# williamyang1991/VToonify

Hardware: AMD Instinct MI355X
Metric: frames/sec at 1024x1024 VToonify-D inference (higher is better)
Workload: dtype bf16

## Files before the change

### __graft_entry__.py

```python
from __future__ import annotations

import json
import os
import sys

REPO = os.path.dirname(os.path.abspath(__file__))
if REPO not in sys.path:
    sys.path.insert(0, REPO)


def build() -> None:
    from vtoonify_amd import build as vbuild
    path = vbuild.build(verbose=False)
    assert os.path.exists(path), path
    sys.path.insert(0, os.path.join(REPO, "tests"))
    from emu import build_emu
    build_emu.build()
    import torch
    from vtoonify_amd import _lib
    import ctypes
    lib = ctypes.CDLL(path)
    for sym in _lib.EXPORTED_SYMBOLS:
        getattr(lib, sym)
    import vtoonify_amd.op
    import vtoonify_amd.vtoonify
    print(f"[build] {path} ok ({len(_lib.EXPORTED_SYMBOLS)} symbols)")


def smoke() -> None:
    import numpy as np
    import torch

    from oracle import vtoonify_oracle as O
    from vtoonify_amd import _lib, synth
    from vtoonify_amd.engine import VToonifyEngine

    assert torch.cuda.is_available(), "smoke() needs a GPU"
# ... 27 lines not shown
```

### include/vtoonify_amd.h

```cpp
#ifndef VTOONIFY_AMD_H
#define VTOONIFY_AMD_H

#include <stdint.h>

#ifdef __cplusplus
extern "C" {
#endif

#define VT_ABI_VERSION 5

enum { VT_F32 = 0, VT_BF16 = 1, VT_F16 = 2,
       VT_F32X3 = 3,
       VT_F64 = 4 };
enum { VT_OK = 0, VT_ERR_ARG = 1, VT_ERR_UNSUPPORTED = 2, VT_ERR_LAUNCH = 3 };

enum { VT_ACT_NONE = 0, VT_ACT_LRELU = 1, VT_ACT_RELU_TANH = 2, VT_ACT_SIGMOID = 3, VT_ACT_TANH = 4  };
enum { VT_OUT_NHWC = 0, VT_OUT_NCHW = 1 };

typedef void* vt_stream;

int vt_abi_version(void);
const char* vt_last_error(void);
const char* vt_build_target(void);

// ... 159 lines not shown
int vt_coords_from_flow(float* coords, const float* flow, int n, int h, int w, vt_stream stream);
int vt_convex_upsample(float* out, const float* flow, const float* mask, int n, int h, int w, vt_stream stream);

int vt_nchw_to_nhwc(void* out, int ld_out, const void* in, int n, int c, int hw,
                    int in_dtype, int out_dtype, vt_stream stream);
int vt_nhwc_to_nchw(void* out, const void* in, int ld_in, int n, int c, int hw,
                    int in_dtype, int out_dtype, vt_stream stream);

int vt_mfma_selftest(float* c, const void* a, const void* b, int dtype, vt_stream stream);

#ifdef __cplusplus
}
#endif

#include "vtoonify_amd_prepass.h"
#endif
```

### vtoonify_amd/_lib.py

```python
from __future__ import annotations

import ctypes as C
import os

HERE = os.path.dirname(os.path.abspath(__file__))
DEFAULT_LIB = os.path.join(HERE, "lib", "libvtoonify_amd.so")

ABI_VERSION = 5
VT_F32, VT_BF16, VT_F16 = 0, 1, 2
VT_F64 = 4
VT_F32X3 = 3
ACT_NONE, ACT_LRELU, ACT_RELU_TANH, ACT_SIGMOID, ACT_TANH = 0, 1, 2, 3, 4
OUT_NHWC, OUT_NCHW = 0, 1


class VtError(RuntimeError):
    pass


class ConvDesc(C.Structure):
    _fields_ = [
        ("src0", C.c_void_p), ("src1", C.c_void_p),
        ("c0", C.c_int32), ("c1", C.c_int32), ("ld0", C.c_int32), ("ld1", C.c_int32),
        ("n", C.c_int32), ("h", C.c_int32), ("w", C.c_int32),
# ... 104 lines not shown
                                 C.c_int, C.c_int, C.c_int, C.c_int, C.c_void_p]),
    "vt_nchw_to_nhwc": (C.c_int, [C.c_void_p, C.c_int, C.c_void_p, C.c_int, C.c_int, C.c_int, C.c_int,
                                  C.c_int, C.c_void_p]),
    "vt_nhwc_to_nchw": (C.c_int, [C.c_void_p, C.c_void_p, C.c_int, C.c_int, C.c_int, C.c_int, C.c_int,
                                  C.c_int, C.c_void_p]),
    "vt_mfma_selftest": (C.c_int, [C.c_void_p, C.c_void_p, C.c_void_p, C.c_int, C.c_void_p]),
}

EXPORTED_SYMBOLS = tuple(_SIGS)

_PREPASS_SIGS = {
    "vt_frame_ingest2x": (C.c_int, [C.c_void_p] * 4 + [C.c_int] * 4 + [C.c_void_p]),
}
PREPASS_SYMBOLS = tuple(_PREPASS_SIGS)

_lib = None
_lib_path = None


def _bind(path: str):
    import torch
    lib = C.CDLL(path)
    for name, (res, args) in {**_SIGS, **_PREPASS_SIGS}.items():
        fn = getattr(lib, name)
        fn.restype = res
        fn.argtypes = args
    if lib.vt_abi_version() != ABI_VERSION:
        raise VtError(f"{path}: ABI version {lib.vt_abi_version()} != {ABI_VERSION}")
    return lib


def use_library(path: str):
    global _lib, _lib_path
    _lib = _bind(path)
    _lib_path = path
    return _lib


# ... 35 lines not shown
```

### vtoonify_amd/build.py

```python
from __future__ import annotations

import os
import shutil
import subprocess
import sys
from concurrent.futures import ThreadPoolExecutor

HERE = os.path.dirname(os.path.abspath(__file__))
CSRC = os.path.join(HERE, "csrc")
LIBDIR = os.path.join(HERE, "lib")
LIBNAME = "libvtoonify_amd.so"
SOURCES = ["capi.hip", "fused_bias_act.hip", "upfirdn2d.hip", "style_ops.hip", "conv_igemm.hip",
           "norm_glue.hip", "frame_io.hip", "parsing_glue.hip", "raft_corr.hip", "flow_ops.hip"]
ARCH = "gfx950"
FLAGS = [f"--offload-arch={ARCH}", "-O3", "-std=c++17", "-fPIC", "-fno-gpu-rdc", "-Wno-unused-result", "-ffp-contract=off",
         "-fno-slp-vectorize"]


def hipcc_path() -> str:
    for cand in (os.environ.get("HIPCC"), shutil.which("hipcc"), "/opt/rocm/bin/hipcc"):
        if cand and os.path.exists(cand):
            return cand
    raise RuntimeError("hipcc not found (ROCm toolchain required to build libvtoonify_amd.so)")


def lib_path() -> str:
    return os.path.join(LIBDIR, LIBNAME)


def _deps(src: str):
    hdrs = [os.path.join(CSRC, f) for f in os.listdir(CSRC) if f.endswith(".hpp")]
    hdrs.append(os.path.join(os.path.dirname(HERE), "include", "vtoonify_amd.h"))
    return [src] + hdrs


def _stale(target: str, deps) -> bool:
    if not os.path.exists(target):
        return True
    t = os.path.getmtime(target)
    return any(os.path.getmtime(d) > t for d in deps)


def _stamp(hipcc: str, flags) -> str:
    import hashlib
    try:
        ver = subprocess.run([hipcc, "--version"], capture_output=True, text=True).stdout
    except OSError:
# ... 74 lines not shown
```

### vtoonify_amd/csrc/conv_igemm.hip

```cpp
#include <stdlib.h>
#include <type_traits>
#include <utility>

#include "vt_common.hpp"

namespace {

#ifdef VT_EMU
typedef emu_f32x4 f32x4;
#else
typedef float f32x4 __attribute__((ext_vector_type(4)));
typedef __bf16 bf16x8_t __attribute__((ext_vector_type(8)));
typedef _Float16 f16x8_t __attribute__((ext_vector_type(8)));
#endif

static inline int slab_ld(int cout_total) { return (cout_total + 31) / 32 * 32; }
constexpr int64_t VT_TICKET_BYTES = 16384;

struct ConvArgs {
    const void* src0;
    const void* src1;
    const void* wgt;
    const float* bias;
    const float* slope_vec;
// ... 22 lines not shown
    int force_generic;
    StatRec* stats_part;
    int post_relu;
    const void* wstream;
    float* tile_stats;
    const float* in_tile_stats;
    int in_stats_dil;
    const float* in_gb;
    int in_ld_gb;
    const float* up_fir;
    int rgb_only;
    int in_absdiff;
    int x3;
    int blk_pm, blk_cn;
    int stride_x, dil_x;
};

static inline bool axes_equal(const ConvArgs& a) { return a.stride_x == a.stride && a.dil_x == a.dil && a.pad_x == a.pad; }

template <typename T>
struct Mma;
template <>
struct Mma<bf16_t> {
    static __device__ __forceinline__ void run(f32x4& acc, const u128& a, const u128& b) {
#ifdef VT_EMU
        emu_bf16x8 av, bv;
        memcpy(&av, &a, 16);
        memcpy(&bv, &b, 16);
        acc = emu_mfma_f32_16x16x32_bf16(av, bv, acc);
#else
// ... 2519 lines not shown
extern "C" int vt_conv2d(const vt_conv_desc* d, vt_stream stream) {
    ConvArgs a;
    const int rc = fill_args(d, a);
    if (rc != VT_OK) return rc;
    const int64_t wsf = (d->splitk_ws && d->splitk_ws_bytes > VT_TICKET_BYTES) ? (d->splitk_ws_bytes - VT_TICKET_BYTES) / 4 : 0;
    g_stats_emitted = false;
    a.x3 = d->dtype == VT_F32X3;
    const int rcl = d->dtype == VT_F16    ? dispatch<f16_t>(a, d->tile_hint, wsf, stream)
                    : d->dtype == VT_BF16 ? dispatch<bf16_t>(a, d->tile_hint, wsf, stream)
                                          : dispatch<float>(a, d->tile_hint, wsf, stream);
    if (rcl != VT_OK || !a.stats_part || g_stats_emitted || d->splitk_phase == 1) return rcl;
    return vt_internal_instnorm_partial(a.stats_part, d->out, d->ld_out, d->n, d->out_h * d->out_w, d->cout,
                                        d->dtype == VT_F32X3 ? VT_F32 : d->dtype, stream);
}

extern "C" int vt_conv2d_tile(const vt_conv_desc* d) {
    ConvArgs a;
    if (fill_args(d, a) != VT_OK) return -1;
    a.force_generic = d->tile_hint >= 1000000000 || !axes_equal(a);
    const int64_t wsf = (d->splitk_ws && d->splitk_ws_bytes > VT_TICKET_BYTES) ? (d->splitk_ws_bytes - VT_TICKET_BYTES) / 4 : 0;
    const TilePlan t = plan_of(d, a, wsf);
    int kind = t.kind;
    if (kind == 0) {
        GldsArgs g;
        const bool glds = d->dtype == VT_F16    ? glds_eligible<f16_t>(a, g)
                          : d->dtype == VT_BF16 ? glds_eligible<bf16_t>(a, g)
                                                : glds_eligible<float>(a, g);
        kind = glds ? 2 : 0;
    }
    int bm = t.bm, bn = t.bn;
// ... 95 lines not shown
```

### vtoonify_amd/csrc/conv_thin.hpp

```cpp
#pragma once

constexpr int TH_TW = 8;
constexpr int TH_NW = 4;
constexpr int TH_MAXF = 7;
constexpr int TH_COLS = 32;
constexpr int TH_PADC = 4;

template <typename T>
static bool thin_eligible(const ConvArgs& a) {
    constexpr int KSTEP = 4 * (16 / (int)sizeof(T));
    if (a.force_generic || !axes_equal(a) || a.transposed || a.rgb_w || a.stats_part || a.tile_stats || a.in_tile_stats || a.up_fir || a.slope_vec)
        return false;
    if (a.in_scale && !a.in_shift) return false;
    if ((a.in_scale || a.in_absdiff) && !(a.taps == 9 && a.taps * a.coutT <= 16)) return false;
    if (a.out_layout != VT_OUT_NCHW || a.phases != 1 || a.stride != 1 || a.dil != 1) return false;
    if (!((a.taps == 9 && a.kw == 3 && a.pad == 1) || (a.taps == 1 && a.pad == 0))) return false;
    if (a.coutT < 1 || a.coutT > 3 || a.taps * a.coutT > TH_COLS) return false;
    if (a.in_absdiff ? (a.c1 != a.c0 || !a.src1 || a.ld1 % (16 / (int)sizeof(T)) != 0 || (uintptr_t)a.src1 % 16 != 0) : a.c1 != 0)
        return false;
    if (a.c0 % KSTEP != 0 || a.ld0 % (16 / (int)sizeof(T)) != 0) return false;
    if (a.Ho != a.H || a.Wo != a.W) return false;
    if ((uintptr_t)a.src0 % 16 != 0 || (uintptr_t)a.wgt % 16 != 0) return false;
    return (int64_t)a.N * a.H * a.W * a.ld0 * (int64_t)sizeof(T) < ((int64_t)1 << 40);
}

__device__ __forceinline__ int thin_tile_of_block() {
    const int nb = (int)gridDim.x, b = (int)blockIdx.x;
    const int q = nb >> 3, r = nb & 7;
    const int xcd = b & 7, idx = b >> 3;
    return (xcd < r ? xcd * (q + 1) : r * (q + 1) + (xcd - r) * q) + idx;
}

template <typename T, int KS, int NB, bool PRO = false>
__global__ void __launch_bounds__(TH_NW * 64) conv_thin_kernel(const ConvArgs p) {
    constexpr int VEC = 16 / (int)sizeof(T);
    constexpr int KSTEP = 4 * VEC;
    constexpr int PW = TH_TW + KS - 1;
    constexpr int NPIX = PW * PW;
    constexpr int NF = (NPIX + 15) / 16;
    constexpr int TAPS = KS * KS;
    constexpr int UNR = KS == 3 ? 3 : 4;
    __shared__ __attribute__((aligned(16))) float dpart[TH_NW][NF * 16][16 * NB + TH_PADC];

    const int tid = threadIdx.x;
    const int lane = tid & 63;
    const int wave = vt_uniform(tid >> 6) & (TH_NW - 1);
    const int q = lane >> 4, l15 = lane & 15;
    const int tiles_x = (p.W + TH_TW - 1) / TH_TW, tiles_y = (p.H + TH_TW - 1) / TH_TW;
    const int tile = thin_tile_of_block();
    const int img = tile / (tiles_x * tiles_y);
    const int trem = tile - img * (tiles_x * tiles_y);
    const int y0 = (trem / tiles_x) * TH_TW, x0 = (trem % tiles_x) * TH_TW;
    const int ncols = TAPS * p.coutT;

    const T* src = (const T*)p.src0;
    const T* oth = (const T*)p.src1;
    int64_t poff[NF], qoff[PRO ? NF : 1];
// ... 113 lines not shown
#pragma unroll
            for (int f = 0; f < NF; ++f) affine(fa[f], poff[f] >= 0, scv, shv, &fo[f]);
#pragma unroll
            for (int f = 0; f < NF; ++f)
#pragma unroll
                for (int b = 0; b < NB; ++b) Mma<T>::run(acc[f][b], fw[b], fa[f]);
        }
    }
#pragma unroll
    for (int f = 0; f < NF; ++f)
#pragma unroll
        for (int b = 0; b < NB; ++b) {
            float v4[4] = {acc[f][b][0], acc[f][b][1], acc[f][b][2], acc[f][b][3]};
            st128(&dpart[wave][f * 16 + l15][b * 16 + q * 4], pack16<float>(v4));
        }
    __syncthreads();

    const int opix = tid & 63, co = tid >> 6;
    const int oy = opix / TH_TW, ox = opix - oy * TH_TW;
    const int gy = y0 + oy, gx = x0 + ox;
    if (co >= p.coutT || gy >= p.H || gx >= p.W) return;
    float s = 0.0f;
#pragma unroll
    for (int tap = 0; tap < TAPS; ++tap) {
        const int ky = tap / KS, kx = tap - ky * KS;
        const int pp = (oy + ky) * PW + ox + kx;
        float t = 0.0f;
#pragma unroll
        for (int w = 0; w < TH_NW; ++w) t += dpart[w][pp][tap * p.coutT + co];
        s += t;
    }
    const float ga = p.gain_alpha * (p.alpha_dev ? p.alpha_dev[0] : 1.0f);
    const float v = conv_finish(p, s, p.bias ? p.bias[co] : 0.0f, ga, p.slope);
    const int64_t HoWo = (int64_t)p.H * p.W;
    const int64_t off = ((int64_t)img * p.cout + co) * HoWo + (int64_t)gy * p.W + gx;
    const float* rs = (const float*)p.resid;
    ((float*)p.out)[off] = post_act(p, v + (rs ? p.beta * rs[off] : 0.0f));
}

constexpr int TH16 = 16;
constexpr int TH16_NW = 4;

template <typename T, int KS, int NB, bool PRO = false>
__global__ void __launch_bounds__(TH16_NW * 64) conv_thin16_kernel(const ConvArgs p) {
    constexpr int VEC = 16 / (int)sizeof(T);
    constexpr int KSTEP = 4 * VEC;
    constexpr int PW = TH16 + KS - 1;
    constexpr int NPIX = PW * PW;
    constexpr int NF = (NPIX + 15) / 16;
    constexpr int FPW = (NF + TH16_NW - 1) / TH16_NW;
    constexpr int TAPS = KS * KS;
    constexpr int UNR = 2;
    __shared__ __attribute__((aligned(16))) float dt[NF * 16][16 * NB + TH_PADC];

    const int tid = threadIdx.x;
    const int lane = tid & 63;
    const int wave = vt_uniform(tid >> 6) & (TH16_NW - 1);
    const int q = lane >> 4, l15 = lane & 15;
    const int tiles_x = (p.W + TH16 - 1) / TH16, tiles_y = (p.H + TH16 - 1) / TH16;
    const int tile = thin_tile_of_block();
    const int img = tile / (tiles_x * tiles_y);
    const int trem = tile - img * (tiles_x * tiles_y);
    const int y0 = (trem / tiles_x) * TH16, x0 = (trem % tiles_x) * TH16;
    const int ncols = TAPS * p.coutT;

    const T* src = (const T*)p.src0;
    const T* oth = (const T*)p.src1;
    int64_t poff[FPW], qoff[PRO ? FPW : 1];
// ... 105 lines not shown
                    for (int b = 0; b < NB; ++b) Mma<T>::run(acc[i][b], fw[u][b], fa[u][i]);
            }
        }
    }
#pragma unroll
    for (int i = 0; i < FPW; ++i) {
        const int f = wave + TH16_NW * i;
        if (f < NF) {
#pragma unroll
            for (int b = 0; b < NB; ++b) {
                float v4[4] = {acc[i][b][0], acc[i][b][1], acc[i][b][2], acc[i][b][3]};
                st128(&dt[f * 16 + l15][b * 16 + q * 4], pack16<float>(v4));
            }
        }
    }
    __syncthreads();
    if (tid >= TH16 * TH16) return;
    const int oy = tid / TH16, ox = tid - oy * TH16;
    const int gy = y0 + oy, gx = x0 + ox;
    if (gy >= p.H || gx >= p.W) return;
    const float ga = p.gain_alpha * (p.alpha_dev ? p.alpha_dev[0] : 1.0f);
    const int64_t HoWo = (int64_t)p.H * p.W;
    const float* rs = (const float*)p.resid;
    for (int co = 0; co < p.coutT; ++co) {
        float s = 0.0f;
#pragma unroll
        for (int tap = 0; tap < TAPS; ++tap) {
            const int ky = tap / KS, kx = tap - ky * KS;
            s += dt[(oy + ky) * PW + ox + kx][tap * p.coutT + co];
        }
        const float v = conv_finish(p, s, p.bias ? p.bias[co] : 0.0f, ga, p.slope);
        const int64_t off = ((int64_t)img * p.cout + co) * HoWo + (int64_t)gy * p.W + gx;
        ((float*)p.out)[off] = post_act(p, v + (rs ? p.beta * rs[off] : 0.0f));
    }
}

static bool thin16_wanted(const ConvArgs& a) {
    return a.taps == 9 && (int64_t)vt_cdiv(a.H, TH16) * vt_cdiv(a.W, TH16) >= 256;
}

template <typename T>
int launch_thin(const ConvArgs& a, vt_stream stream) {
    ConvArgs args = a;
    args.splitk = 1;
    args.kps = 0;
    const int64_t blocks = (int64_t)a.N * vt_cdiv(a.H, TH_TW) * vt_cdiv(a.W, TH_TW);
    if (blocks >= ((int64_t)1 << 31)) {
        vt_set_error("vt_conv2d: too many tiles");
        return VT_ERR_ARG;
    }
    const bool two = a.taps * a.coutT > 16;
    if ((a.in_scale || a.in_absdiff) && (a.taps != 9 || two)) {
        vt_set_error("vt_conv2d: in_scale / in_absdiff on a thin conv need a 3x3 kernel with 9 * cout <= 16");
        return VT_ERR_UNSUPPORTED;
    }
    if (thin16_wanted(a)) {
        const unsigned b16 = (unsigned)((int64_t)a.N * vt_cdiv(a.H, TH16) * vt_cdiv(a.W, TH16));
        if (a.in_scale || a.in_absdiff) {
            auto k = conv_thin16_kernel<T, 3, 1, true>;
            VT_LAUNCH(k, dim3(b16), dim3(TH16_NW * 64), stream, args);
        } else if (two) {
            auto k = conv_thin16_kernel<T, 3, 2>;
            VT_LAUNCH(k, dim3(b16), dim3(TH16_NW * 64), stream, args);
        } else {
            auto k = conv_thin16_kernel<T, 3, 1>;
            VT_LAUNCH(k, dim3(b16), dim3(TH16_NW * 64), stream, args);
        }
        return vt_check_launch("vt_conv2d(thin, 16x16)");
    }
    if (a.in_scale || a.in_absdiff) {
        auto k = conv_thin_kernel<T, 3, 1, true>;
        VT_LAUNCH(k, dim3((unsigned)blocks), dim3(TH_NW * 64), stream, args);
    } else if (a.taps == 9 && two) {
        auto k = conv_thin_kernel<T, 3, 2>;
        VT_LAUNCH(k, dim3((unsigned)blocks), dim3(TH_NW * 64), stream, args);
    } else if (a.taps == 9) {
        auto k = conv_thin_kernel<T, 3, 1>;
        VT_LAUNCH(k, dim3((unsigned)blocks), dim3(TH_NW * 64), stream, args);
    } else {
        auto k = conv_thin_kernel<T, 1, 1>;
        VT_LAUNCH(k, dim3((unsigned)blocks), dim3(TH_NW * 64), stream, args);
    }
    return vt_check_launch("vt_conv2d(thin)");
// ... 2 lines not shown
```

### vtoonify_amd/engine.py

```python
from __future__ import annotations

import ctypes as C
import math
import os
from typing import Dict, List, Optional, Tuple

import torch

from . import _lib
from . import kernels as K
from ._lib import ACT_LRELU, ACT_NONE, ACT_RELU_TANH, OUT_NCHW, OUT_NHWC

SQRT2 = math.sqrt(2.0)
N_LATENT = 18
_DIL = {1: 4, 2: 4, 3: 2, 4: 2, 5: 1, 6: 1}
FEM_HDR = 64


def _pad8(c: int) -> int:
    return (c + 7) // 8 * 8


class _Plan:
    def __init__(self):
# ... 2 lines not shown
        self.enc_ops: List[Tuple] = []
        self.gen_ops: List[Tuple] = []
        self.keep: list = []
        self.masks: List[torch.Tensor] = []
        self.graphs: dict = {}
        self.convs: list = []


class VToonifyEngine:
    supports_borrow = True

    def __init__(self, state_dict: Dict[str, torch.Tensor], backbone: str = "dualstylegan",
                 in_size: int = 256, dtype: torch.dtype = torch.bfloat16,
                 device: Optional[torch.device] = None, cache_styles: bool = False,
                 tile_hints: Optional[Dict[str, int]] = None, style_gate: bool = False, x3: bool = False,
                 fuse_rgb128: bool = True):
        assert backbone in ("dualstylegan", "toonify")
        assert dtype in (torch.bfloat16, torch.float16, torch.float32)
        self.backbone = backbone
        self.dual = backbone == "dualstylegan"
        self.in_size = in_size
        self.dtype = dtype
        self.dt = K.dt_code(dtype)
        self.x3 = bool(x3) and dtype == torch.float32
        self.dt_conv = K.VT_F32X3 if self.x3 else self.dt
        self.h16 = dtype in (torch.bfloat16, torch.float16)
        self.precision = ({torch.bfloat16: "bf16", torch.float16: "fp16"}[dtype] if self.h16 else
                          ("fp32x3" if self.x3 else "fp32_exact"))
        self.esz = 2 if self.h16 else 4
        any_t = next(iter(state_dict.values()))
        self.device = torch.device(device) if device is not None else any_t.device
        if self.device.type == "cuda" and self.device.index is None:
            self.device = torch.device("cuda", torch.cuda.current_device())
        self.lib = _lib.lib()
        if self.device.type != "cuda" and not _lib.is_emulation():
            raise _lib.VtError("VToonifyEngine needs a GPU device (no CPU path)")
        self.cache_styles = cache_styles
        self.fuse_rgb128 = bool(fuse_rgb128)
        self.style_gate = bool(style_gate)
        self.graph_first = os.environ.get("VT_GRAPH_FIRST", "1") != "0"
        self.use_upblur = True
        self.tile_hints: Dict[str, int] = dict(tile_hints or {})
        if not self.tile_hints and os.environ.get("VT_TILE_HINTS"):
            import json
            with open(os.environ["VT_TILE_HINTS"]) as f:
                self.tile_hints = {k: int(v) for k, v in json.load(f).items()}
        self.sd = {k: v.detach().to(self.device, torch.float32).contiguous() for k, v in state_dict.items()}
        self.g = "generator.generator." if self.dual else "generator."
        self.n_down = 0
        while f"encoder.{self.n_down}.0.weight" in self.sd:
            self.n_down += 1
        self.n_fuse = sum(1 for lvl in range(5) if 2 ** (5 + lvl) <= in_size)
        import collections
# ... 69 lines not shown
        t = torch.empty(shape, dtype=dtype or self.dtype, device=self.device)
        plan.bufs[name] = t
        return t

    @staticmethod
    def conv_signature(d) -> str:
        return (f"{d.h}x{d.w}:{d.c0 + d.c1}->{d.cout * d.phases}:k{d.kh}s{d.stride}d{d.dil}p{d.phases}"
                + (":nchw" if d.out_layout == OUT_NCHW else "") + (":up" if d.up_fir else ""))

    def _apply_hint(self, d):
        h = self.tile_hints.get(self.conv_signature(d))
        if h:
            d.tile_hint = int(h)
        return d

    def _op_conv(self, ops, plan, ref_macs=None, branch=0, join=False, **kw):
        wt = kw.get("weight")
        if isinstance(wt, torch.Tensor) and wt.data_ptr() in self._wstream:
            kw["weight_stream"] = self._wstream[wt.data_ptr()]
        d = self._apply_hint(K.make_conv_desc(dtype=self.dt_conv, **kw))
        plan.keep.append(d)
        cin = d.c0 + d.c1
        m = d.n * d.out_h * d.out_w
        cout_t = d.cout * d.phases
        macs = m * cout_t * d.kh * d.kw * cin if ref_macs is None else ref_macs
        osz = 4 if d.out_dtype == K.VT_F32 else 2
        nbytes = (d.n * d.h * d.w * cin * self.esz + cout_t * d.kh * d.kw * cin * self.esz +
                  m * cout_t * osz * (2 if d.resid else 1))
        info = {"name": "conv", "kernel": "conv_igemm", "flops": 2 * macs, "bytes": nbytes, "cin": cin,
                "cout": cout_t, "m": m, "k": d.kh * d.kw * cin, "hw": (d.out_h, d.out_w),
                "sig": self.conv_signature(d)}
        if branch:
            info["branch"] = branch
        if join:
            info["join"] = True
        plan.convs.append((d, info, ops, len(ops)))
        ops.append((self.lib.vt_conv2d, (C.byref(d),), info))

    def _conv_kind(self, **kw) -> int:
        wt = kw.get("weight")
        if isinstance(wt, torch.Tensor) and wt.data_ptr() in self._wstream:
            kw["weight_stream"] = self._wstream[wt.data_ptr()]
        d = self._apply_hint(K.make_conv_desc(dtype=self.dt_conv, **kw))
        d.splitk_ws, d.splitk_ws_bytes = 1 << 20, 1 << 40
        tile = self.lib.vt_conv2d_tile(C.byref(d))
        return tile // 100000000 if tile >= 0 else -1

    def _op_linear(self, ops, y, ld_y, x, ld_x, W, b, rows, w_scale=1.0, b_scale=1.0, act=ACT_NONE,
                   slope=0.2, gain=1.0):
        out_dim, in_dim = W.shape
        ops.append((self.lib.vt_linear,
# ... 262 lines not shown
        plan.feat = (feat, cf, h, w)
        skip = self._buf(plan, "skip_enc", (B, 3, h, w), f32)
        self._op_conv(ops, plan, src0=feat, c0=cf, ld0=cf, n=B, h=h, w=w, out_h=h, out_w=w,
                      weight=self.w["enc_rgb"], cout=3, kh=1, kw=1, bias=sd[f"encoder.{self.n_down + 1}.bias"],
                      out=skip, ld_out=0, out_layout=OUT_NCHW, out_dtype=K.VT_F32, branch=1)
        plan.skip_enc = skip

        ops = plan.gen_ops
        out, co = feat, cf
        for lvl in range(5):
            hw = h * w
            if lvl < self.n_fuse:
                f_e, ce, he, we = feats[lvl]
                assert (he, we) == (h, w) and ce == co, "encoder/generator size mismatch (H, W must be multiples of 8)"
                fem = self._buf(plan, f"fem{lvl}", (B, h, w, co + FEM_HDR))
                mask = None
                if self.dual:
                    sc = self._buf(plan, f"fsc{lvl}", (B, 2 * co), f32)
                    sh = self._buf(plan, f"fsh{lvl}", (B, 2 * co), f32)
                    ws = self._buf(plan, f"fws{lvl}", (max(K.instnorm_ws_bytes(B, hw, 2 * co), 16),), torch.uint8)
                    gb = plan.bufs[f"gb.fus.{lvl}"]
                    ops.append((lib.vt_instnorm_stats,
                                (C.c_void_p(sc.data_ptr()), C.c_void_p(sh.data_ptr()), C.c_void_p(out.data_ptr()), co,
                                 C.c_void_p(f_e.data_ptr()), co, B, hw, co, C.c_void_p(gb.data_ptr()),
                                 0 if ns == 1 else gb.shape[1], C.c_void_p(ws.data_ptr()), dt),
                                {"name": "instnorm", "kernel": "instnorm_stats", "flops": 0,
                                 "bytes": 2 * B * hw * co * self.esz}))
                    mask = self._buf(plan, f"mask{lvl}", (B, 1, h, w), f32)
                    mask_kw = dict(n=B, h=h, w=w, out_h=h, out_w=w, weight=self.w[f"fusion_out.{lvl}.conv2"], cout=1,
                                   kh=3, kw=3, pad=1, bias=sd[f"fusion_out.{lvl}.conv2.bias"], act=ACT_RELU_TANH,
                                   out=mask, ld_out=0, out_layout=OUT_NCHW, out_dtype=K.VT_F32)
                    gate_kw = dict(src0=out, c0=co, ld0=co, src1=f_e, c1=co, ld1=co, in_scale=sc, in_shift=sh, in_absdiff=1)
                    gl = os.environ.get("VT_GATE_LOADER", "1")
                    in_loader = (gl != "0" and (hw >= 4096 or gl == "2") and self._conv_kind(**gate_kw, **mask_kw) == 6)
                    if in_loader:
                        self._op_conv(ops, plan, **gate_kw, **mask_kw)
                    else:
                        nrm = self._buf(plan, f"nrm{lvl}", (B, h, w, 2 * co))
                        ops.append((lib.vt_affine_apply,
                                    (C.c_void_p(nrm.data_ptr()), 2 * co, C.c_void_p(out.data_ptr()), co,
                                     C.c_void_p(f_e.data_ptr()), co, C.c_void_p(sc.data_ptr()),
                                     C.c_void_p(sh.data_ptr()), B, hw, co, dt),
                                    {"name": "affine", "kernel": "affine_apply", "flops": 0,
                                     "bytes": 4 * B * hw * co * self.esz}))
                        self._op_conv(ops, plan, src0=nrm, c0=2 * co, ld0=2 * co, **mask_kw)
                    plan.masks.append(mask)
                ops.append((lib.vt_fusion_pack,
                            (C.c_void_p(fem.data_ptr()), co + FEM_HDR, C.c_void_p(f_e.data_ptr()), co,
                             C.c_void_p(mask.data_ptr() if mask is not None else 0), C.c_void_p(skip.data_ptr()),
                             B, hw, co, dt),
                            {"name": "fusion_pack", "kernel": "fusion_pack", "flops": 0, "join": True,
                             "bytes": B * hw * (co * self.esz + (co + FEM_HDR) * self.esz + 16)}))
                fo = self._buf(plan, f"fout{lvl}", (B, h, w, co))
                wkey = f"fusion_out.{lvl}.conv" if self.dual else f"fusion_out.{lvl}"
                self._op_conv(ops, plan, src0=out, c0=co, ld0=co, src1=fem.data_ptr() + FEM_HDR * self.esz, c1=co,
                              ld1=co + FEM_HDR, n=B, h=h, w=w, out_h=h, out_w=w, weight=self.w[wkey], cout=co, kh=3,
                              kw=3, pad=1, bias=sd[wkey + ".bias"], out=fo, ld_out=co)
                sk2 = self._buf(plan, f"fskip{lvl}", (B, 3, h, w), f32)
                self._op_conv(ops, plan, src0=fem, c0=co + FEM_HDR, ld0=co + FEM_HDR, n=B, h=h, w=w, out_h=h, out_w=w,
                              weight=self.w[f"fusion_skip.{lvl}"], cout=3, kh=3, kw=3, pad=1,
                              bias=sd[f"fusion_skip.{lvl}.bias"], out=sk2, ld_out=0, out_layout=OUT_NCHW,
                              out_dtype=K.VT_F32, branch=1)
                out, skip = fo, sk2
            n1, n2, n3 = f"convs.{6 + 2 * lvl}", f"convs.{7 + 2 * lvl}", f"to_rgbs.{3 + lvl}"
            c1o = self.modw[n1].shape[0]
            up = self._buf(plan, f"up{lvl}", (B, 2 * h, 2 * w, c1o))
            o2 = self._buf(plan, f"gout{lvl}", (B, 2 * h, 2 * w, c1o))
# ... 60 lines not shown
                plan.bufs["splitk_ws" if br == 0 else f"splitk_ws{br}"] = wss[br]
        tname = {K.VT_BF16: "bf16", K.VT_F16: "f16"}.get(self.dt, "f32")
        inserts = []
        for d, info, ops, pos in plan.convs:
            ws = wss.get(info.get("branch", 0))
            if ws is not None:
                d.splitk_ws, d.splitk_ws_bytes = ws.data_ptr(), ws.numel()
            tile = self.lib.vt_conv2d_tile(C.byref(d))
            if tile < 0:
                raise _lib.VtError(f"vt_conv2d descriptor rejected: {self.lib.vt_last_error().decode()}")
            kind, sk, bm, bn = tile // 100000000, (tile // 1000000) % 100, (tile // 1000) % 1000, tile % 1000
            kname = {0: "conv_igemm_kernel", 1: "conv_patch_kernel", 2: "conv_igemm_glds_kernel",
                     3: "conv3x3_c32_kernel", 4: "conv_fullk_kernel", 5: "conv_upblur_kernel",
                     6: "conv_thin_kernel", 7: "conv_patchs2_kernel", 8: "conv_fullkw_kernel", 9: "conv_upblur_rows_kernel",
                     10: "conv_upflat_kernel"}[kind]
            info["kernel"] = f"{kname}<{tname},{bm}x{bn}>"
            info["splitk"] = sk
            if sk > 1 and self.lib.vt_conv2d_splitk_mode(C.byref(d)) == 2:
                d.splitk_phase = 1
                d2 = _lib.ConvDesc.from_buffer_copy(d)
                d2.splitk_phase = 2
                plan.keep.append(d2)
                m, cout_t = info["m"], info["cout"]
                osz = 4 if d.out_dtype == K.VT_F32 else 2
                rk = "conv_splitk_reduce_stats_kernel" if d.stats_part else "conv_splitk_reduce_kernel"
                rinfo = {"name": "splitk_reduce", "kernel": rk, "flops": 0,
                         "bytes": sk * m * ((cout_t + 7) // 8 * 8) * 4 + m * cout_t * osz}
                if info.get("branch"):
                    rinfo["branch"] = info["branch"]
                inserts.append((ops, pos, (self.lib.vt_conv2d, (C.byref(d2),), rinfo)))
# ... 188 lines not shown
```

### vtoonify_amd/kernels.py

```python
from __future__ import annotations

import ctypes as C

import torch

from . import _lib
from ._lib import ACT_LRELU, ACT_NONE, ACT_RELU_TANH, OUT_NCHW, OUT_NHWC, VT_BF16, VT_F16, VT_F32, VT_F32X3, VT_F64, ConvDesc

_DT = {torch.float32: VT_F32, torch.bfloat16: VT_BF16, torch.float16: VT_F16}


def dt_code(dtype: torch.dtype) -> int:
    try:
        return _DT[dtype]
    except KeyError:
        raise _lib.VtError(f"unsupported dtype {dtype}") from None


def op_dt_code(dtype: torch.dtype) -> int:
    return VT_F64 if dtype == torch.float64 else dt_code(dtype)


def _dev_ok(*tensors):
    for t in tensors:
# ... 208 lines not shown
    def ptr(v):
        return C.c_void_p(0 if v is None else (v.data_ptr() if isinstance(v, torch.Tensor) else int(v)))
    t = stream_of if stream_of is not None else scale
    _lib.check(_lib.lib().vt_affine_apply(ptr(out), ld_out, ptr(x), ld_x, ptr(other), ld_other, ptr(scale),
                                         ptr(shift), n, hw, c, dtype, _stream(t)), "vt_affine_apply")


def fusion_pack(out, ld_out, f_e, ld_e, mask, skip, n, hw, c, dtype, stream_of=None):
    def ptr(v):
        return C.c_void_p(0 if v is None else (v.data_ptr() if isinstance(v, torch.Tensor) else int(v)))
    t = stream_of if stream_of is not None else skip
    _lib.check(_lib.lib().vt_fusion_pack(ptr(out), ld_out, ptr(f_e), ld_e, ptr(mask), ptr(skip), n, hw, c,
                                        dtype, _stream(t)), "vt_fusion_pack")


def nchw_to_nhwc(x: torch.Tensor, out_dtype, ld_out=None, out=None):
    _dev_ok(x)
    n, c, h, w = x.shape
    cpad = (c + 7) // 8 * 8
    ld_out = ld_out or cpad
    if out is None:
        out = torch.empty((n, h, w, ld_out), dtype=out_dtype, device=x.device)
    _lib.check(_lib.lib().vt_nchw_to_nhwc(_p(out), ld_out, _p(x), n, c, h * w, dt_code(x.dtype),
                                         dt_code(out.dtype), _stream(x)), "vt_nchw_to_nhwc")
    return out


def nhwc_to_nchw(x_ptr, ld_in, n, c, h, w, in_dtype, out_dtype, device, stream_of):
    out = torch.empty((n, c, h, w), dtype=out_dtype, device=device)
    ptr = x_ptr.data_ptr() if isinstance(x_ptr, torch.Tensor) else int(x_ptr)
# ... 24 lines not shown
```

Baseline: 1670.

## Fuse fusion_pack into the thin gate mask conv epilogue

Adds a PACK variant of the thin-output conv kernels. After computing the per-pixel gate mask, it writes the masked encoder features, the skip RGB header and the zero padding straight into the fem buffer, so the separate fusion_pack kernel launch can be dropped. This removes one launch and one extra read of the mask and encoder features per fusion level. In exchange it adds a second block barrier, shared-memory staging of the mask and more register pressure in the thin kernel, and it only applies when the gate uses the in-loader thin path.

```diff
diff --git a/__graft_entry__.py b/__graft_entry__.py
--- a/__graft_entry__.py
+++ b/__graft_entry__.py
@@ -20,7 +20,7 @@
     from vtoonify_amd import _lib
     import ctypes
     lib = ctypes.CDLL(path)
-    for sym in _lib.EXPORTED_SYMBOLS:
+    for sym in _lib.EXPORTED_SYMBOLS + _lib.PREPASS_SYMBOLS + _lib.GATE_SYMBOLS:
         getattr(lib, sym)
     import vtoonify_amd.op
     import vtoonify_amd.vtoonify
diff --git a/include/vtoonify_amd.h b/include/vtoonify_amd.h
--- a/include/vtoonify_amd.h
+++ b/include/vtoonify_amd.h
@@ -197,4 +197,5 @@
 #endif
 
 #include "vtoonify_amd_prepass.h"
+#include "vtoonify_amd_gate.h"
 #endif
diff --git a/include/vtoonify_amd_gate.h b/include/vtoonify_amd_gate.h
--- /dev/null
+++ b/include/vtoonify_amd_gate.h
@@ -0,0 +1,14 @@
+#ifndef VTOONIFY_AMD_GATE_H
+#define VTOONIFY_AMD_GATE_H
+#include "vtoonify_amd.h"
+
+#ifdef __cplusplus
+extern "C" {
+#endif
+
+int vt_fusion_gate(const vt_conv_desc* d, void* fem, int ld_fem, const float* skip, vt_stream stream);
+
+#ifdef __cplusplus
+}
+#endif
+#endif
diff --git a/vtoonify_amd/_lib.py b/vtoonify_amd/_lib.py
--- a/vtoonify_amd/_lib.py
+++ b/vtoonify_amd/_lib.py
@@ -142,6 +142,11 @@
 }
 PREPASS_SYMBOLS = tuple(_PREPASS_SIGS)
 
+_GATE_SIGS = {
+    "vt_fusion_gate": (C.c_int, [C.POINTER(ConvDesc), C.c_void_p, C.c_int, C.c_void_p, C.c_void_p]),
+}
+GATE_SYMBOLS = tuple(_GATE_SIGS)
+
 _lib = None
 _lib_path = None
 
@@ -149,7 +154,7 @@
 def _bind(path: str):
     import torch
     lib = C.CDLL(path)
-    for name, (res, args) in {**_SIGS, **_PREPASS_SIGS}.items():
+    for name, (res, args) in {**_SIGS, **_PREPASS_SIGS, **_GATE_SIGS}.items():
         fn = getattr(lib, name)
         fn.restype = res
         fn.argtypes = args
diff --git a/vtoonify_amd/build.py b/vtoonify_amd/build.py
--- a/vtoonify_amd/build.py
+++ b/vtoonify_amd/build.py
@@ -30,7 +30,8 @@
 
 def _deps(src: str):
     hdrs = [os.path.join(CSRC, f) for f in os.listdir(CSRC) if f.endswith(".hpp")]
-    hdrs.append(os.path.join(os.path.dirname(HERE), "include", "vtoonify_amd.h"))
+    inc = os.path.join(os.path.dirname(HERE), "include")
+    hdrs += [os.path.join(inc, f) for f in sorted(os.listdir(inc)) if f.endswith(".h")]
     return [src] + hdrs
 
 
diff --git a/vtoonify_amd/csrc/conv_igemm.hip b/vtoonify_amd/csrc/conv_igemm.hip
--- a/vtoonify_amd/csrc/conv_igemm.hip
+++ b/vtoonify_amd/csrc/conv_igemm.hip
@@ -60,6 +60,9 @@
     int x3;
     int blk_pm, blk_cn;
     int stride_x, dil_x;
+    void* fem;
+    const float* skip;
+    int ld_fem;
 };
 
 static inline bool axes_equal(const ConvArgs& a) { return a.stride_x == a.stride && a.dil_x == a.dil && a.pad_x == a.pad; }
@@ -2609,6 +2612,31 @@
                                         d->dtype == VT_F32X3 ? VT_F32 : d->dtype, stream);
 }
 
+extern "C" int vt_fusion_gate(const vt_conv_desc* d, void* fem, int ld_fem, const float* skip, vt_stream stream) {
+    ConvArgs a;
+    const int rc = fill_args(d, a);
+    if (rc != VT_OK) return rc;
+    VT_REQUIRE(fem && skip, "vt_fusion_gate: null tensor");
+    const int esz = (d->dtype == VT_F32 || d->dtype == VT_F32X3) ? 4 : 2;
+    VT_REQUIRE(ld_fem >= d->c0 + 8 && (ld_fem - d->c0) % 8 == 0 && (uintptr_t)fem % 16 == 0 && (int64_t)ld_fem * esz % 16 == 0,
+               "vt_fusion_gate: bad fem (ld_fem = header + c0, header a multiple of 8, >= 8; 16-byte aligned rows)");
+    if (!(a.in_absdiff && a.coutT == 1 && a.phases == 1 && a.taps == 9 && a.kw == 3 && a.pad == 1 && a.out_layout == VT_OUT_NCHW &&
+          a.out_f32 && !a.resid && !a.stats_part && !a.rgb_w)) {
+        vt_set_error("vt_fusion_gate: needs the Fusion gate's mask conv (in_absdiff, cout 1, 3x3, pad 1, fp32 NCHW output, no residual)");
+        return VT_ERR_UNSUPPORTED;
+    }
+    a.force_generic = d->tile_hint >= 1000000000 || !axes_equal(a);
+    const int64_t wsf = (d->splitk_ws && d->splitk_ws_bytes > VT_TICKET_BYTES) ? (d->splitk_ws_bytes - VT_TICKET_BYTES) / 4 : 0;
+    if (plan_of(d, a, wsf).kind != 6) {
+        vt_set_error("vt_fusion_gate: the descriptor does not run on the thin-output kernel");
+        return VT_ERR_UNSUPPORTED;
+    }
+    a.fem = fem;
+    a.ld_fem = ld_fem;
+    a.skip = skip;
+    return d->dtype == VT_F16 ? launch_thin<f16_t>(a, stream) : d->dtype == VT_BF16 ? launch_thin<bf16_t>(a, stream) : launch_thin<float>(a, stream);
+}
+
 extern "C" int vt_conv2d_tile(const vt_conv_desc* d) {
     ConvArgs a;
     if (fill_args(d, a) != VT_OK) return -1;
diff --git a/vtoonify_amd/csrc/conv_thin.hpp b/vtoonify_amd/csrc/conv_thin.hpp
--- a/vtoonify_amd/csrc/conv_thin.hpp
+++ b/vtoonify_amd/csrc/conv_thin.hpp
@@ -31,7 +31,87 @@
     return (xcd < r ? xcd * (q + 1) : r * (q + 1) + (xcd - r) * q) + idx;
 }
 
-template <typename T, int KS, int NB, bool PRO = false>
+template <typename T, int TW>
+struct ThinPack {
+    static constexpr int VEC = 16 / (int)sizeof(T);
+    static constexpr int NPX = TW * TW, NT = 256, UNR = 8;
+    int px, cv, dpx, dcv, cvn;
+    u128 fr[UNR];
+    int64_t off[UNR];
+    int mp[UNR];
+
+    __device__ __forceinline__ void load(const ConvArgs& p, int img, int y0, int x0) {
+        const T* fe = (const T*)p.src1;
+        const int hdr = p.ld_fem - p.c0;
+        const u128 zero = u128{0u, 0u, 0u, 0u};
+#pragma unroll
+        for (int u = 0; u < UNR; ++u) {
+            const int gy = y0 + px / TW, gx = x0 + px % TW;
+            const bool ok = px < NPX && gy < p.H && gx < p.W;
+            const int64_t pix = ((int64_t)img * p.H + gy) * p.W + gx;
+            fr[u] = ok ? ld128(fe + pix * p.ld1 + cv * VEC) : zero;
+            off[u] = pix * p.ld_fem + hdr + cv * VEC;
+            mp[u] = ok ? px : -1;
+            cv += dcv;
+            px += dpx;
+            if (cv >= cvn) cv -= cvn, ++px;
+        }
+    }
+
+    __device__ __forceinline__ void start(const ConvArgs& p, int img, int y0, int x0, int tid) {
+        T* fem = (T*)p.fem;
+        const int64_t HW = (int64_t)p.H * p.W;
+        const int hv = (p.ld_fem - p.c0) / VEC;
+        const int gy = y0 + tid / TW, gx = x0 + tid % TW;
+        const bool in = tid < NPX && gy < p.H && gx < p.W;
+        const int64_t pl = (int64_t)gy * p.W + gx;
+        float h[VEC];
+#pragma unroll
+        for (int k = 0; k < VEC; ++k) h[k] = (k < 3 && in) ? p.skip[((int64_t)img * 3 + k) * HW + pl] : 0.0f;
+        cvn = p.c0 / VEC;
+        px = tid / cvn;
+        cv = tid - px * cvn;
+        dpx = NT / cvn;
+        dcv = NT - dpx * cvn;
+        load(p, img, y0, x0);
+        const int hz = hv - 1;
+        if (hz > 0) {
+            float z[VEC];
+#pragma unroll
+            for (int k = 0; k < VEC; ++k) z[k] = 0.0f;
+            const u128 zv = pack16<T>(z);
+            int qx = tid / hz, v = tid - qx * hz;
+            const int dq = NT / hz, dv = NT - dq * hz;
+            for (; qx < NPX;) {
+                const int zy = y0 + qx / TW, zx = x0 + qx % TW;
+                if (zy < p.H && zx < p.W) st128(fem + (((int64_t)img * p.H + zy) * p.W + zx) * p.ld_fem + (v + 1) * VEC, zv);
+                v += dv;
+                qx += dq;
+                if (v >= hz) v -= hz, ++qx;
+            }
+        }
+        if (in) st128(fem + ((int64_t)img * HW + pl) * p.ld_fem, pack16<T>(h));
+    }
+
+    __device__ __forceinline__ void finish(const ConvArgs& p, const float* mk, int img, int y0, int x0) {
+        T* fem = (T*)p.fem;
+        for (;;) {
+#pragma unroll
+            for (int u = 0; u < UNR; ++u) {
+                float f[VEC];
+                unpack16<T>(fr[u], f);
+                const float m = mk[mp[u] >= 0 ? mp[u] : 0];
+#pragma unroll
+                for (int k = 0; k < VEC; ++k) f[k] *= m;
+                if (mp[u] >= 0) st128(fem + off[u], pack16<T>(f));
+            }
+            if (px >= NPX) break;
+            load(p, img, y0, x0);
+        }
+    }
+};
+
+template <typename T, int KS, int NB, bool PRO = false, bool PACK = false>
 __global__ void __launch_bounds__(TH_NW * 64) conv_thin_kernel(const ConvArgs p) {
     constexpr int VEC = 16 / (int)sizeof(T);
     constexpr int KSTEP = 4 * VEC;
@@ -41,6 +121,7 @@
     constexpr int TAPS = KS * KS;
     constexpr int UNR = KS == 3 ? 3 : 4;
     __shared__ __attribute__((aligned(16))) float dpart[TH_NW][NF * 16][16 * NB + TH_PADC];
+    __shared__ float mk[PACK ? TH_TW * TH_TW : 1];
 
     const int tid = threadIdx.x;
     const int lane = tid & 63;
@@ -184,34 +265,47 @@
             float v4[4] = {acc[f][b][0], acc[f][b][1], acc[f][b][2], acc[f][b][3]};
             st128(&dpart[wave][f * 16 + l15][b * 16 + q * 4], pack16<float>(v4));
         }
+    ThinPack<T, TH_TW> pk;
+    if constexpr (PACK) pk.start(p, img, y0, x0, tid);
     __syncthreads();
 
     const int opix = tid & 63, co = tid >> 6;
     const int oy = opix / TH_TW, ox = opix - oy * TH_TW;
     const int gy = y0 + oy, gx = x0 + ox;
-    if (co >= p.coutT || gy >= p.H || gx >= p.W) return;
-    float s = 0.0f;
-#pragma unroll
-    for (int tap = 0; tap < TAPS; ++tap) {
-        const int ky = tap / KS, kx = tap - ky * KS;
-        const int pp = (oy + ky) * PW + ox + kx;
-        float t = 0.0f;
-#pragma unroll
-        for (int w = 0; w < TH_NW; ++w) t += dpart[w][pp][tap * p.coutT + co];
-        s += t;
-    }
-    const float ga = p.gain_alpha * (p.alpha_dev ? p.alpha_dev[0] : 1.0f);
-    const float v = conv_finish(p, s, p.bias ? p.bias[co] : 0.0f, ga, p.slope);
-    const int64_t HoWo = (int64_t)p.H * p.W;
-    const int64_t off = ((int64_t)img * p.cout + co) * HoWo + (int64_t)gy * p.W + gx;
-    const float* rs = (const float*)p.resid;
-    ((float*)p.out)[off] = post_act(p, v + (rs ? p.beta * rs[off] : 0.0f));
+    const bool mine = co < p.coutT && gy < p.H && gx < p.W;
+    if constexpr (!PACK) {
+        if (!mine) return;
+    }
+    if (!PACK || mine) {
+        float s = 0.0f;
+#pragma unroll
+        for (int tap = 0; tap < TAPS; ++tap) {
+            const int ky = tap / KS, kx = tap - ky * KS;
+            const int pp = (oy + ky) * PW + ox + kx;
+            float t = 0.0f;
+#pragma unroll
+            for (int w = 0; w < TH_NW; ++w) t += dpart[w][pp][tap * p.coutT + co];
+            s += t;
+        }
+        const float ga = p.gain_alpha * (p.alpha_dev ? p.alpha_dev[0] : 1.0f);
+        const float v = conv_finish(p, s, p.bias ? p.bias[co] : 0.0f, ga, p.slope);
+        const int64_t HoWo = (int64_t)p.H * p.W;
+        const int64_t off = ((int64_t)img * p.cout + co) * HoWo + (int64_t)gy * p.W + gx;
+        const float* rs = (const float*)p.resid;
+        const float r = post_act(p, v + (rs ? p.beta * rs[off] : 0.0f));
+        ((float*)p.out)[off] = r;
+        if constexpr (PACK) mk[opix] = r;
+    }
+    if constexpr (PACK) {
+        __syncthreads();
+        pk.finish(p, mk, img, y0, x0);
+    }
 }
 
 constexpr int TH16 = 16;
 constexpr int TH16_NW = 4;
 
-template <typename T, int KS, int NB, bool PRO = false>
+template <typename T, int KS, int NB, bool PRO = false, bool PACK = false>
 __global__ void __launch_bounds__(TH16_NW * 64) conv_thin16_kernel(const ConvArgs p) {
     constexpr int VEC = 16 / (int)sizeof(T);
     constexpr int KSTEP = 4 * VEC;
@@ -222,6 +316,7 @@
     constexpr int TAPS = KS * KS;
     constexpr int UNR = 2;
     __shared__ __attribute__((aligned(16))) float dt[NF * 16][16 * NB + TH_PADC];
+    __shared__ float mk[PACK ? TH16 * TH16 : 1];
 
     const int tid = threadIdx.x;
     const int lane = tid & 63;
@@ -357,24 +452,36 @@
             }
         }
     }
+    ThinPack<T, TH16> pk;
+    if constexpr (PACK) pk.start(p, img, y0, x0, tid);
     __syncthreads();
-    if (tid >= TH16 * TH16) return;
     const int oy = tid / TH16, ox = tid - oy * TH16;
     const int gy = y0 + oy, gx = x0 + ox;
-    if (gy >= p.H || gx >= p.W) return;
-    const float ga = p.gain_alpha * (p.alpha_dev ? p.alpha_dev[0] : 1.0f);
-    const int64_t HoWo = (int64_t)p.H * p.W;
-    const float* rs = (const float*)p.resid;
-    for (int co = 0; co < p.coutT; ++co) {
-        float s = 0.0f;
-#pragma unroll
-        for (int tap = 0; tap < TAPS; ++tap) {
-            const int ky = tap / KS, kx = tap - ky * KS;
-            s += dt[(oy + ky) * PW + ox + kx][tap * p.coutT + co];
-        }
-        const float v = conv_finish(p, s, p.bias ? p.bias[co] : 0.0f, ga, p.slope);
-        const int64_t off = ((int64_t)img * p.cout + co) * HoWo + (int64_t)gy * p.W + gx;
-        ((float*)p.out)[off] = post_act(p, v + (rs ? p.beta * rs[off] : 0.0f));
+    const bool mine = tid < TH16 * TH16 && gy < p.H && gx < p.W;
+    if constexpr (!PACK) {
+        if (!mine) return;
+    }
+    if (!PACK || mine) {
+        const float ga = p.gain_alpha * (p.alpha_dev ? p.alpha_dev[0] : 1.0f);
+        const int64_t HoWo = (int64_t)p.H * p.W;
+        const float* rs = (const float*)p.resid;
+        for (int co = 0; co < p.coutT; ++co) {
+            float s = 0.0f;
+#pragma unroll
+            for (int tap = 0; tap < TAPS; ++tap) {
+                const int ky = tap / KS, kx = tap - ky * KS;
+                s += dt[(oy + ky) * PW + ox + kx][tap * p.coutT + co];
+            }
+            const float v = conv_finish(p, s, p.bias ? p.bias[co] : 0.0f, ga, p.slope);
+            const int64_t off = ((int64_t)img * p.cout + co) * HoWo + (int64_t)gy * p.W + gx;
+            const float r = post_act(p, v + (rs ? p.beta * rs[off] : 0.0f));
+            ((float*)p.out)[off] = r;
+            if constexpr (PACK) mk[tid] = r;
+        }
+    }
+    if constexpr (PACK) {
+        __syncthreads();
+        pk.finish(p, mk, img, y0, x0);
     }
 }
 
@@ -397,8 +504,17 @@
         vt_set_error("vt_conv2d: in_scale / in_absdiff on a thin conv need a 3x3 kernel with 9 * cout <= 16");
         return VT_ERR_UNSUPPORTED;
     }
+    if (a.fem && !(a.in_absdiff && a.coutT == 1 && a.taps == 9)) {
+        vt_set_error("vt_fusion_gate: the pack tail needs the in_absdiff mask conv (3x3, cout 1)");
+        return VT_ERR_UNSUPPORTED;
+    }
     if (thin16_wanted(a)) {
         const unsigned b16 = (unsigned)((int64_t)a.N * vt_cdiv(a.H, TH16) * vt_cdiv(a.W, TH16));
+        if (a.fem) {
+            auto k = conv_thin16_kernel<T, 3, 1, true, true>;
+            VT_LAUNCH(k, dim3(b16), dim3(TH16_NW * 64), stream, args);
+            return vt_check_launch("vt_fusion_gate(thin, 16x16)");
+        }
         if (a.in_scale || a.in_absdiff) {
             auto k = conv_thin16_kernel<T, 3, 1, true>;
             VT_LAUNCH(k, dim3(b16), dim3(TH16_NW * 64), stream, args);
@@ -410,6 +526,11 @@
             VT_LAUNCH(k, dim3(b16), dim3(TH16_NW * 64), stream, args);
         }
         return vt_check_launch("vt_conv2d(thin, 16x16)");
+    }
+    if (a.fem) {
+        auto k = conv_thin_kernel<T, 3, 1, true, true>;
+        VT_LAUNCH(k, dim3((unsigned)blocks), dim3(TH_NW * 64), stream, args);
+        return vt_check_launch("vt_fusion_gate(thin)");
     }
     if (a.in_scale || a.in_absdiff) {
         auto k = conv_thin_kernel<T, 3, 1, true>;
diff --git a/vtoonify_amd/engine.py b/vtoonify_amd/engine.py
--- a/vtoonify_amd/engine.py
+++ b/vtoonify_amd/engine.py
@@ -40,7 +40,7 @@
                  in_size: int = 256, dtype: torch.dtype = torch.bfloat16,
                  device: Optional[torch.device] = None, cache_styles: bool = False,
                  tile_hints: Optional[Dict[str, int]] = None, style_gate: bool = False, x3: bool = False,
-                 fuse_rgb128: bool = True):
+                 fuse_rgb128: bool = True, fuse_gate_pack: bool = True):
         assert backbone in ("dualstylegan", "toonify")
         assert dtype in (torch.bfloat16, torch.float16, torch.float32)
         self.backbone = backbone
@@ -63,6 +63,7 @@
             raise _lib.VtError("VToonifyEngine needs a GPU device (no CPU path)")
         self.cache_styles = cache_styles
         self.fuse_rgb128 = bool(fuse_rgb128)
+        self.fuse_gate_pack = bool(fuse_gate_pack)
         self.style_gate = bool(style_gate)
         self.graph_first = os.environ.get("VT_GRAPH_FIRST", "1") != "0"
         self.use_upblur = True
@@ -162,7 +163,7 @@
             d.tile_hint = int(h)
         return d
 
-    def _op_conv(self, ops, plan, ref_macs=None, branch=0, join=False, **kw):
+    def _op_conv(self, ops, plan, ref_macs=None, branch=0, join=False, gate_pack=None, **kw):
         wt = kw.get("weight")
         if isinstance(wt, torch.Tensor) and wt.data_ptr() in self._wstream:
             kw["weight_stream"] = self._wstream[wt.data_ptr()]
@@ -183,6 +184,14 @@
         if join:
             info["join"] = True
         plan.convs.append((d, info, ops, len(ops)))
+        if gate_pack is not None:
+            fem, ld_fem, skip = gate_pack
+            info.update(pack=True, join=True,
+                        bytes=(d.n * d.h * d.w * cin * self.esz + cout_t * d.kh * d.kw * cin * self.esz + m * cout_t * osz +
+                               m * (ld_fem * self.esz + 12)))
+            ops.append((self.lib.vt_fusion_gate, (C.byref(d), C.c_void_p(fem.data_ptr()), ld_fem, C.c_void_p(skip.data_ptr())),
+                        info))
+            return
         ops.append((self.lib.vt_conv2d, (C.byref(d),), info))
 
     def _conv_kind(self, **kw) -> int:
@@ -475,7 +484,7 @@
                 f_e, ce, he, we = feats[lvl]
                 assert (he, we) == (h, w) and ce == co, "encoder/generator size mismatch (H, W must be multiples of 8)"
                 fem = self._buf(plan, f"fem{lvl}", (B, h, w, co + FEM_HDR))
-                mask = None
+                mask, packed = None, False
                 if self.dual:
                     sc = self._buf(plan, f"fsc{lvl}", (B, 2 * co), f32)
                     sh = self._buf(plan, f"fsh{lvl}", (B, 2 * co), f32)
@@ -494,7 +503,10 @@
                     gate_kw = dict(src0=out, c0=co, ld0=co, src1=f_e, c1=co, ld1=co, in_scale=sc, in_shift=sh, in_absdiff=1)
                     gl = os.environ.get("VT_GATE_LOADER", "1")
                     in_loader = (gl != "0" and (hw >= 4096 or gl == "2") and self._conv_kind(**gate_kw, **mask_kw) == 6)
-                    if in_loader:
+                    packed = in_loader and self.fuse_gate_pack
+                    if packed:
+                        self._op_conv(ops, plan, gate_pack=(fem, co + FEM_HDR, skip), **gate_kw, **mask_kw)
+                    elif in_loader:
                         self._op_conv(ops, plan, **gate_kw, **mask_kw)
                     else:
                         nrm = self._buf(plan, f"nrm{lvl}", (B, h, w, 2 * co))
@@ -506,12 +518,13 @@
                                      "bytes": 4 * B * hw * co * self.esz}))
                         self._op_conv(ops, plan, src0=nrm, c0=2 * co, ld0=2 * co, **mask_kw)
                     plan.masks.append(mask)
-                ops.append((lib.vt_fusion_pack,
-                            (C.c_void_p(fem.data_ptr()), co + FEM_HDR, C.c_void_p(f_e.data_ptr()), co,
-                             C.c_void_p(mask.data_ptr() if mask is not None else 0), C.c_void_p(skip.data_ptr()),
-                             B, hw, co, dt),
-                            {"name": "fusion_pack", "kernel": "fusion_pack", "flops": 0, "join": True,
-                             "bytes": B * hw * (co * self.esz + (co + FEM_HDR) * self.esz + 16)}))
+                if not packed:
+                    ops.append((lib.vt_fusion_pack,
+                                (C.c_void_p(fem.data_ptr()), co + FEM_HDR, C.c_void_p(f_e.data_ptr()), co,
+                                 C.c_void_p(mask.data_ptr() if mask is not None else 0), C.c_void_p(skip.data_ptr()),
+                                 B, hw, co, dt),
+                                {"name": "fusion_pack", "kernel": "fusion_pack", "flops": 0, "join": True,
+                                 "bytes": B * hw * (co * self.esz + (co + FEM_HDR) * self.esz + 16)}))
                 fo = self._buf(plan, f"fout{lvl}", (B, h, w, co))
                 wkey = f"fusion_out.{lvl}.conv" if self.dual else f"fusion_out.{lvl}"
                 self._op_conv(ops, plan, src0=out, c0=co, ld0=co, src1=fem.data_ptr() + FEM_HDR * self.esz, c1=co,
@@ -602,6 +615,8 @@
                      3: "conv3x3_c32_kernel", 4: "conv_fullk_kernel", 5: "conv_upblur_kernel",
                      6: "conv_thin_kernel", 7: "conv_patchs2_kernel", 8: "conv_fullkw_kernel", 9: "conv_upblur_rows_kernel",
                      10: "conv_upflat_kernel"}[kind]
+            if info.get("pack"):
+                kname = "conv_thin_pack_kernel"
             info["kernel"] = f"{kname}<{tname},{bm}x{bn}>"
             info["splitk"] = sk
             if sk > 1 and self.lib.vt_conv2d_splitk_mode(C.byref(d)) == 2:
diff --git a/vtoonify_amd/kernels.py b/vtoonify_amd/kernels.py
--- a/vtoonify_amd/kernels.py
+++ b/vtoonify_amd/kernels.py
@@ -246,6 +246,15 @@
                                         dtype, _stream(t)), "vt_fusion_pack")
 
 
+def fusion_gate(fem, ld_fem, skip, *, stream_of=None, **kw):
+    d = make_conv_desc(**kw)
+    t = stream_of
+    if t is None:
+        t = kw["out"] if isinstance(kw["out"], torch.Tensor) else skip
+    _lib.check(_lib.lib().vt_fusion_gate(C.byref(d), C.c_void_p(_ptr(fem)), int(ld_fem), C.c_void_p(_ptr(skip)), _stream(t)),
+               "vt_fusion_gate")
+
+
 def nchw_to_nhwc(x: torch.Tensor, out_dtype, ld_out=None, out=None):
     _dev_ok(x)
     n, c, h, w = x.shape
```

Result: no change. 1664 (-0.4%).
